# peterdavidfagan/mujoco_robot_environments

Measured on AMD Instinct MI355X. Metric: env steps/sec (whole node), RearrangementEnv batch=4096 at 1/2/4/8 MI355X, higher is better.
Workload: dtype f32

## Files before the change

mujoco_robot_environments_amd/csrc/mre_api.cpp:

```cpp
#include <hip/hip_runtime.h>
#include <chrono>

#include <cmath>
#include <cstdio>
#include <cstdlib>
#include <cstring>
#include <string>
#include <algorithm>
#include <vector>

#include "../../include/mre.h"
#include "mre_dev.h"
#include "mre_records.h"

using namespace mre;

extern "C" void mre_launch_step(const StepArgs* args, hipStream_t stream);
extern "C" void mre_launch_settle(const StepArgs* args, hipStream_t stream);
extern "C" void mre_launch_step_large(const StepArgs* args, hipStream_t stream);
extern "C" void mre_launch_step_newton(const StepArgs* args, hipStream_t stream);
extern "C" void mre_launch_settle_newton(const StepArgs* args, hipStream_t stream);
extern "C" void mre_launch_step_queue(const StepArgs* args, int nwaves, hipStream_t stream);
extern "C" void mre_launch_step_queue_newton(const StepArgs* args, int nwaves, hipStream_t stream);
extern "C" void mre_launch_step_queue_large(const StepArgs* args, int nwaves, hipStream_t stream);
// ... 87 lines not shown
  std::vector<uint8_t> h_large, h_rerun;
  int n_large = 0;
  long long* d_env_ids = nullptr;
  int *ps_attempts = nullptr, *ps_prop = nullptr, *ps_tick = nullptr, *ps_which = nullptr;
  double *ps_bounds = nullptr, *ps_pose = nullptr, *ps_zones = nullptr, *ps_pick = nullptr;
  int prop_geom0 = 12;
  int last_settle_max = 0;
  long long n_reruns = 0, n_promotions = 0, n_demotions = 0;
  struct Group {
    int lo = 0, n = 0;
    hipStream_t st = nullptr, st2 = nullptr;
    hipEvent_t ev_fork = nullptr, ev_join = nullptr;
    struct Out {
      StepArgs args;
      hipEvent_t ev_info = nullptr;
      int stage = 0;
    } out[4];
    int head = 0, nout = 0;
    int cur = 0;
    hipEvent_t p0 = nullptr, p1 = nullptr;
    int* h_order = nullptr;
    int* d_order = nullptr;
  };
  std::vector<Group> groups;
  int* h_grp_order = nullptr;
  int* d_grp_order = nullptr;
  Group qgroup;
  bool queue_ok = true;
  int queue_ticks = 200;
  int queue_waves = 0;
  int queue_shards = 16;
  int queue_lshards = 8;
  bool queue_test_serial = false;
  int queue_spare_large = 8;
  int queue_run_ticks = 100;
  int queue_min_ticks = 32;
  float tick_tail = 0.f;
  bool tick_tail_valid = false;
  float queue_tail_min = 1.45f;
  unsigned tail_samples = 0;
  std::vector<int> tail_scratch;
  int queue_large_waves_max = 0;
  int* h_qlist = nullptr;
  int* q_ws = nullptr;
  int* q_gen = nullptr;
  int* h_q_err = nullptr;
  int* h_qgrp_order = nullptr;
  long n_queue_launches = 0;
  long long n_handovers = 0;
  int queue_last_handovers = 0;
  static constexpr int RING = 4;
  int ring = 2;
  static constexpr int NSTAGE = RING + 1;
  static_assert(sizeof(Group::out) / sizeof(Group::Out) == RING, "Group::out is the ring");
  hipEvent_t ev_main = nullptr;
  float* seq_copy[RING + 1] = {nullptr, nullptr, nullptr, nullptr, nullptr};
  size_t seq_cap = 0;
  unsigned seq_calls = 0;
  double dbg_wait_s = 0, dbg_call_s = 0; long dbg_calls = 0;
  int calls_since_drain = 0, sync_streak = 0;
  bool broken = false;
};

static void launch_compact(const mre_env* e, const StepArgs& a, hipStream_t st, bool settle = false) {
  const bool newton = e->hM.solver == MRE_SOLVER_NEWTON;
  if (settle) { if (newton) mre_launch_settle_newton(&a, st); else mre_launch_settle(&a, st); }
  else { if (newton) mre_launch_step_newton(&a, st); else mre_launch_step(&a, st); }
}
static void launch_large(const mre_env* e, const StepArgs& a, hipStream_t st) {
  if (e->hM.solver == MRE_SOLVER_NEWTON) mre_launch_step_large_newton(&a, st); else mre_launch_step_large(&a, st);
}

static int profile_events(mre_env* e, hipEvent_t* e0, hipEvent_t* e1) {
  *e0 = *e1 = nullptr;
  if (!e->profiling) return MRE_OK;
  if (e->events_used == e->events.size()) {
    hipEvent_t x, y;
    HIPCHK(hipEventCreate(&x)); HIPCHK(hipEventCreate(&y));
    e->events.emplace_back(x, y);
  }
  *e0 = e->events[e->events_used].first; *e1 = e->events[e->events_used].second;
  e->events_used++;
  return MRE_OK;
}

static inline int compact_nrrow_max(const mre_env* e) {
  return e->hM.solver == MRE_SOLVER_NEWTON ? NRROW_MAX_COMPACT_NEWTON : NRROW_MAX_COMPACT_PGS;
}
static inline bool near_compact_caps(const mre_env* e, int hw_ncon, int hw_nefc, int hw_nrrow, int hw_npp) {
  return 8 * hw_ncon > 7 * NCON_MAX || 8 * hw_nefc > 7 * NEFC_MAX || 8 * hw_nrrow > 7 * compact_nrrow_max(e) || 8 * hw_npp > 7 * NPP_MAX;
}

static void sort_longest_first(const mre_env::Group& G, const int* info, int kmax, int* order_stage) {
  int count[258] = {0};
  auto bucket = [&](int i) {
    const int* li = info + 4 * (size_t)i;
    return (int)((long long)(li[0] < 0 ? 0 : (li[1] >> 16)) * 255 / kmax);
  };
  for (int i = G.lo; i < G.lo + G.n; i++) count[255 - bucket(i) + 1]++;
  for (int k = 1; k <= 256; k++) count[k] += count[k - 1];
  for (int i = G.lo; i < G.lo + G.n; i++) order_stage[G.lo + count[255 - bucket(i)]++] = i;
}
// ... 119 lines not shown
    if (rc) return rc;
  }
  return drain_group(e, e->qgroup, true);
}
#define DRAIN(e) do { int rc_ = drain(e, true); if (rc_) return rc_; } while (0)
#define DRAIN_PENDING(e) do { int rc_ = drain(e, false); if (rc_) return rc_; } while (0)

static void guard_args(mre_env* e, StepArgs& a) {
  a.large = e->d_large; a.launch_info = e->d_launch_info;
  a.sv_qpos = e->sv_qpos; a.sv_qvel = e->sv_qvel; a.sv_qacc_ws = e->sv_qacc_ws; a.sv_qfine = e->sv_qfine;
  a.sv_ctrl = e->sv_ctrl; a.sv_status = e->sv_status; a.sv_converged = e->sv_converged; a.sv_nstep = e->sv_nstep;
}

static int launch_group_enqueue(mre_env* e, mre_env::Group& G, const StepArgs& a_full, bool queue);
static int launch_group(mre_env* e, mre_env::Group& G, const StepArgs& a_full, bool queue = false) {
  const int keep = a_full.nsteps <= 50 ? e->ring - 1 : 0;
  while (G.nout > keep) {
    int rc = process_oldest(e, G);
    if (rc) return rc;
  }
  int rc = launch_group_enqueue(e, G, a_full, queue);
  if (rc) {
    (void)hipStreamSynchronize(G.st);
    (void)hipStreamSynchronize(G.st2);
    G.nout = 0; G.head = 0;
    (void)hipMemset(e->d_pending + G.lo, 0, (size_t)G.n);
    e->broken = true;
  }
  return rc;
}
static int launch_group_enqueue(mre_env* e, mre_env::Group& G, const StepArgs& a_full, bool queue) {
  int rc;
  StepArgs a = a_full;
  const size_t N = (size_t)e->N;
  if (G.nout == 0) {
    memcpy(e->h_large_stage + (size_t)G.cur * N + G.lo, e->h_large.data() + G.lo, (size_t)G.n);
    int kmax = 0;
    for (int i = G.lo; i < G.lo + G.n; i++) {
      const int* li = e->h_info_last + 4 * (size_t)i;
      if (li[0] >= 0 && (li[1] >> 16) > kmax) kmax = li[1] >> 16;
    }
    if (kmax > 0) sort_longest_first(G, e->h_info_last, kmax, G.h_order + (size_t)G.cur * N);
  }
  a.N = G.n; a.env_order = G.d_order + (size_t)G.cur * N + G.lo; a.seq_stride = e->N;
  rc = profile_events(e, &G.p0, &G.p1);
  if (rc) return rc;
  HIPCHK(hipStreamWaitEvent(G.st, e->ev_main, 0));
  if (G.p0) HIPCHK(hipEventRecord(G.p0, G.st));
  guard_args(e, a);
  a.pending = e->d_pending;
  const int slot = (G.head + G.nout) % mre_env::RING;
  a.large = e->d_large_stage + (size_t)G.cur * N;
  a.launch_info = e->d_launch_info + (size_t)slot * 4 * N;
  StepArgs ac = a;
  ac.want_large = 0;
  bool run_large = false;
  const uint8_t* const fl = e->h_large_stage + (size_t)G.cur * N;
  if (queue) {
    const int nt = a.nsteps / a.control_steps, S = e->queue_shards, cap = (G.n + S - 1) / S;
    const int SL = e->queue_lshards, capl = (G.n + SL - 1) / SL;
    constexpr int QS = QUEUE_SHARDS_MAX + QUEUE_LSHARDS_MAX;
    const size_t ctl = 2 * (size_t)QS * QUEUE_TICKS_MAX + 16;
    const size_t stride = (size_t)S * cap + (size_t)SL * capl;
    const size_t words = ctl + 4 * N + (size_t)nt * stride;
    ac.sv_qpos = nullptr;
    ac.q_head = e->q_ws; ac.q_tail = ac.q_head + QS * QUEUE_TICKS_MAX;
// ... 710 lines not shown
      e->queue_large_waves_max = 2 * prop.multiProcessorCount;
      if (const char* q = getenv("MRE_QUEUE_LSHARDS")) { const int v = atoi(q); if (v >= 1 && v <= QUEUE_LSHARDS_MAX) e->queue_lshards = v; }
      HIPCHK(hipMalloc(&e->q_ws, ((2 * (size_t)(QUEUE_SHARDS_MAX + QUEUE_LSHARDS_MAX) * QUEUE_TICKS_MAX + 16 + 4 * N +
                                   (size_t)QUEUE_TICKS_MAX * (2 * N + QUEUE_SHARDS_MAX + QUEUE_LSHARDS_MAX)) * 4 + 15) / 16 * 16));
      HIPCHK(hipMalloc(&e->q_gen, 64));
      HIPCHK(hipMemsetAsync(e->q_gen, 0, 64, e->stream));
      HIPCHK(hipHostMalloc((void**)&e->h_qlist, (size_t)(mre_env::RING + 1) * (N + 32) * 4, hipHostMallocDefault));
      HIPCHK(hipHostMalloc((void**)&e->h_q_err, 64, hipHostMallocMapped | hipHostMallocCoherent));
      *e->h_q_err = 0;
    }
    for (int g = 0; g < ng; g++) {
      auto& G = e->groups[g];
      G.h_order = e->h_grp_order; G.d_order = e->d_grp_order;
      G.lo = (int)((long long)num_envs * g / ng);
      G.n = (int)((long long)num_envs * (g + 1) / ng) - G.lo;
      int pr = 0;
      {
        int least = 0, greatest = 0;
        HIPCHK(hipDeviceGetStreamPriorityRange(&least, &greatest));
        const char* gp = getenv("MRE_GROUP_PRIORITY");
        if (!(gp && atoi(gp) == 0)) { pr = greatest + g; if (pr > least) pr = least; }
        if (const char* map = getenv("MRE_GROUP_PRIO_MAP")) {
          if ((int)strlen(map) > g && map[g] >= '0' && map[g] <= '9') { pr = greatest + (map[g] - '0'); if (pr > least) pr = least; }
        }
      }
      HIPCHK(hipStreamCreateWithPriority(&G.st, hipStreamNonBlocking, pr));
      HIPCHK(hipStreamCreateWithPriority(&G.st2, hipStreamNonBlocking, pr));
      HIPCHK(hipEventCreateWithFlags(&G.ev_fork, hipEventDisableTiming));
      HIPCHK(hipEventCreateWithFlags(&G.ev_join, hipEventDisableTiming));
      for (auto& o : G.out) HIPCHK(hipEventCreateWithFlags(&o.ev_info, hipEventDisableTiming));
    }
  }
  if (const char* fb = getenv("MRE_NO_FALLBACK")) e->fallback = atoi(fb) == 0;
  if (const char* fl = getenv("MRE_FORCE_LARGE")) {
    if (atoi(fl) != 0) {
      e->h_large.assign(N, 1); e->n_large = num_envs;
      HIPCHK(hipMemsetAsync(e->d_large, 1, N, e->stream));
    }
  }
  HIPCHK(hipMemsetAsync(e->status, 0, N * 4, e->stream)); HIPCHK(hipMemsetAsync(e->stats, 0, N * 16, e->stream));
  HIPCHK(hipMemsetAsync(e->grip_closed, 0, N, e->stream)); HIPCHK(hipMemsetAsync(e->osc_target, 0, N * 64, e->stream));
  HIPCHK(hipMemsetAsync(e->sites, 0, N * 64, e->stream));
  std::vector<int> np(N, NPROP);
  std::vector<float> ps(N * NPROP * 3, 0.0155f);
  HIPCHK(hipMemcpy(e->nprops, np.data(), N * 4, hipMemcpyHostToDevice));
  HIPCHK(hipMemcpy(e->prop_size, ps.data(), ps.size() * 4, hipMemcpyHostToDevice));
  e->osc = OscConfig{350.f, 20.f, 500.f, 100.f, 200.f, 30.f, {0.f, -0.785f, 0.f, -2.356f, 0.f, 1.571f, 0.785f},
                     5e-3f, 68e-3f, 0};
  HIPCHK(hipMalloc(&e->d_osc, sizeof(OscConfig)));
  HIPCHK(hipMemcpy(e->d_osc, &e->osc, sizeof(OscConfig), hipMemcpyHostToDevice));
  HIPCHK(hipStreamSynchronize(e->stream));
  int rc = mre_reset(e, nullptr);
  if (rc != MRE_OK) return rc;
  return mre_sync(e);
}

extern "C" int mre_create(const void* blob, size_t nbytes, int num_envs, int device_id, mre_env** out) {
  if (!blob || !out || num_envs <= 0) return fail(MRE_ERR_ARG, "mre_create: bad argument");
  *out = nullptr;
  mre_env* e = new mre_env();
  int rc = build_model(blob, nbytes, e->hM);
  if (rc != MRE_OK) { delete e; return rc; }
  if (const char* it = getenv("MRE_DEBUG_ITERS")) e->hM.iterations = atoi(it);
  e->prop_geom0 = -1;
  for (int g = 0; g < NG; g++) if (e->hM.geom_propid[g] == 0) e->prop_geom0 = g;
  if (e->prop_geom0 != PROP_GEOM0 || e->hM.geom_type[1] != 1 || e->hM.geom_body[1] != 0) {
// ... 1120 lines not shown
```

mujoco_robot_environments_amd/csrc/mre_dev.h:

```cpp
#pragma once
#include <stdint.h>

namespace mre {

constexpr int NB = 20;
constexpr int NRB = 16;
constexpr int GRIP_BODY0 = 8;
constexpr int NV = 39;
constexpr int NRV = 15;
constexpr int NQ = 43;
constexpr int NQP = 44;
constexpr int TRACE_W = 88;
constexpr int TRACE_QVEL = 48;
constexpr int NVP = 40;
constexpr int NU = 8;
constexpr int QFINE = 32;
constexpr int QFINE_ROW = 96;
constexpr int QFINE_CUBE_Q = 32;
constexpr int QFINE_CUBE_V = 60;
static_assert(QFINE_CUBE_Q + 7 * 4 == QFINE_CUBE_V && QFINE_CUBE_V + 6 * 4 <= QFINE_ROW, "qfine row layout");
constexpr int NPROP = 4;
constexpr int NG = 20;
constexpr int PROP_GEOM0 = 12;
constexpr int NPAIR = 128;
// ... 148 lines not shown
  float site_pos[NSITE][3], site_quat[NSITE][4];
  int eef_site, tcp_site;
  int eq_type[NEQ], eq_obj[NEQ][2];
  float eq_data[NEQ][8], eq_solref[NEQ][2], eq_solimp[NEQ][5];
  int ten_dof[2];
  float ten_coef[2];
  int act_dof[NU];
  float act_ctrlrange[NU][2], grip_gainprm, grip_biasprm[3], grip_forcerange[2];
  float act_gain[NU], act_bias[NU][3], act_forcerange[NU][2];
  int act_forcelimited[NU];
  float timestep, gravity[3], impratio, tolerance;
  int iterations;
  int solver;
  int cone;
  float home_qpos[7];
  float park_pos[NPROP][3];
  BodyRec body_rec[NB];
  DofRec dof_rec[NV];
  MEntryRec m_rec[NMR];
  RowRec row_rec[NROWREC];
  EqRec eq_rec[NEQ];
  SiteRec site_rec[NSITE];
  OptRec opt_rec;
};

struct OscConfig {
  float kp_pos, kd_pos, kp_ori, kd_ori, kp_null, kd_null;
  float null_q[7];
  float pos_thresh, ori_thresh;
  int pinv_always;
};

enum StepFlags : unsigned { F_NO_CONSTRAINTS = 1u, F_FREEZE_ROBOT = 2u, F_CONV_CONTINUE = 4u, F_CONV_OPEN = 8u,
                            F_OSC_EVAL = 16u, F_DETECT = 32u, F_SETTLE_EXIT = 64u };
enum CtrlMode : int { CTRL_HELD = 0, CTRL_SEQ = 1, CTRL_OSC = 2 };

struct StepArgs {
  const DevModel* M;
  int N;
  float* qpos;
  float* qvel;
  float* qacc_ws;
  float* qfine;
  float* ctrl;
  const float* ctrl_seq;
  int seq_stride;
  const int* nprops;
  const float* prop_size;
  int nsteps, control_steps, mode;
  unsigned flags;
  const OscConfig* osc;
  int osc_stride;
  const float* osc_target;
  const uint8_t* grip_closed;
  uint8_t* converged;
  float* sites;
  uint32_t* status;
  int* nstep;
  int* stats;
  float* trace;
  int trace_nenv, trace_max, trace_base;
  const uint8_t* env_mask;
  const int* env_order;
  float* geoms;
  float* contacts;
  int* settle_steps;
  int min_settle_steps;
// ... 87 lines not shown
```

mujoco_robot_environments_amd/csrc/mre_kernels.hip:

```cpp
#include <hip/hip_runtime.h>

#include "mre_dev.h"
#include "mre_math.h"
#include "mre_collide.h"

namespace mre {
using ModelP = MRE_MODEL_PTR(DevModel);
#if defined(MRE_PHASE_STAMPS) && MRE_PHASE_STAMPS >= 4
__shared__ unsigned long long dbg_acc[4];
#endif

struct OscSm {
  float J[6][7], M[7][7], MiJt[7][6], Li[6][6], Lam[6][6], V[6][6], Jbar[7][6];
  float ep[3], eo[3], F[6], LF[6], tn[7], Jbt[6], xd[6], w[6];
};

struct alignas(8) Blk {
  uint16_t row0;
  uint8_t type, nrows;
  uint8_t rslot;
  uint8_t pa, pb;
  uint8_t primary : 4;
  uint8_t bslot : 4;
};
// ... 36 lines not shown
  union { float scratch[64]; int iscr[64]; };
  float osc_tgt[16];
  int nprops;
  int ncon, nefc, nl, nrrow, npp, overflow, solver_iters;
  int finger_contact;
  uint8_t con_pair[NCON_MAX], con_rslot[NCON_MAX], con_bslot[NCON_MAX], con_b1[NCON_MAX], con_b2[NCON_MAX];
  uint16_t lim_info[NRV + 1];
  union {
    float JpA[3 * NCON_MAX][6];
    struct {
      float cinert[NB][10], crb[NRB][10], gP[NRB - GRIP_BODY0][6], gC[NRB - GRIP_BODY0][6];
      double gpose[NRB - GRIP_BODY0][7];
    };
  };
  float JpB[3 * NPP_MAX][6];
  union {
    float Jr[NRROW_MAX][NRV];
    struct {
      float cdof_dot[NV][6], cvel[NB][6], cfrc[NB][6];
      alignas(8) double gI[NRB - GRIP_BODY0][10];
      double gS[NRB - GRIP_BODY0][6];
    };
  };
#ifdef MRE_NEWTON
  float efc_R[NEFC_MAX], efc_aref[NEFC_MAX];
  float frc_r[NRROW_MAX];
  float con_fric[NCON_MAX];
  float hc[NCON_MAX][6];
  float Md[NRV][MD_LD];
  alignas(8) float W[NV * (NV + 1) / 2];
  uint8_t rstate[NEFC_MAX];
  uint8_t clist[NPROP][NCON_MAX];
  uint8_t ccount[NPROP], cpl_robot, cpl_cubes;
  alignas(8) uint16_t jdesc[NEFC_MAX][4];
  float zrow[24];
#else
  float Br[NRROW_MAX][NRV];
  alignas(16) float blkrec[MAXBLK][16];
  Blk blk[MAXBLK];
  uint8_t sched[MAXBLK][8];
#endif
  uint16_t hdr[NEFC_MAX];

  int nblk, nsched;
};

#if defined(MRE_LARGE_CAPS)
static_assert(sizeof(Sm) <= 27136, "large-capacity Sm must fit 6 workgroups per CU");
#else
static_assert(sizeof(Sm) <= 20480, "compact Sm must fit 8 workgroups per CU");
#endif

#ifdef MRE_NEWTON
MRE_DEV float* mh_store(Sm& s) { return &s.JpA[0][0]; }
static_assert(sizeof(((Sm*)0)->JpA) >= sizeof(float) * NMR, "M - h dF/dv fits the head of the constraint block");
#else
MRE_DEV float* mh_store(Sm& s) { return s.qLD; }
#endif

struct BodyRegs {
  float anchor[3], axis[3], xipos[3], ximat[9];
};

MRE_DEV double robot_q(const Sm& s, int d) { return (double)s.qpos[d] + (double)s.qlo[d]; }
MRE_DEV double robot_v(const Sm& s, int d) { return (double)s.qvel[d] + (double)s.qlo[QFINE / 2 + d]; }

// ... 1204 lines not shown
    const float v = a.qpos[(size_t)env * NQP + l];
    s.qpos[l] = v;
    if (save) a.sv_qpos[(size_t)env * NQP + l] = v;
  }
  if (l < NVP) {
    const float v = a.qvel[(size_t)env * NVP + l], w = a.qacc_ws[(size_t)env * NVP + l];
    s.qvel[l] = v;
    s.qacc[l] = w;
    s.qfrc_con[l] = 0.f;
    if (save) { a.sv_qvel[(size_t)env * NVP + l] = v; a.sv_qacc_ws[(size_t)env * NVP + l] = w; }
  }
  if (l < QFINE) {
    const float v = a.qfine != nullptr ? a.qfine[(size_t)env * QFINE_ROW + l] : 0.f;
    s.qlo[l] = v;
    if (save && a.qfine != nullptr) a.sv_qfine[(size_t)env * QFINE_ROW + l] = v;
  }
  if (save && a.qfine != nullptr && l < QFINE_ROW - QFINE)
    a.sv_qfine[(size_t)env * QFINE_ROW + QFINE + l] = a.qfine[(size_t)env * QFINE_ROW + QFINE + l];
  float cube_lo_keep = 0.f;
  if (QUEUE && !Q_LARGE && a.qfine != nullptr && l < QFINE_ROW - QFINE) cube_lo_keep = a.qfine[(size_t)env * QFINE_ROW + QFINE + l];
  if (l < NU) {
    const float v = a.ctrl[(size_t)env * NU + l];
    s.ctrl[l] = v;
    if (save) a.sv_ctrl[(size_t)env * NU + l] = v;
  }
  if (save && l == 0) {
    if (a.nstep != nullptr) a.sv_nstep[env] = a.nstep[env];
    a.sv_status[env] = a.status[env];
    a.sv_converged[env] = a.converged != nullptr ? a.converged[env] : (uint8_t)0;
  }
  if (l == 0) { s.nprops = a.nprops[env]; s.overflow = 0; s.ncon = 0; s.nefc = 0; s.solver_iters = 0; }
#ifdef MRE_NEWTON
  if (l < 24) s.zrow[l] = 0.f;
#endif
  if (l < NPROP * 3) {
    const float sz = a.prop_size[(size_t)env * NPROP * 3 + l];
    s.prop_size[l / 3][l % 3] = sz;
  }
  MRE_SYNC();
  if (l < NPROP) {
    const float m = M->body_mass[NRB + l];
    const float* z = s.prop_size[l];
    s.prop_mass[l] = m;
    s.prop_inertia[l][0] = m / 3.f * (z[1] * z[1] + z[2] * z[2]);
    s.prop_inertia[l][1] = m / 3.f * (z[0] * z[0] + z[2] * z[2]);
    s.prop_inertia[l][2] = m / 3.f * (z[0] * z[0] + z[1] * z[1]);
  }
  MRE_SYNC();

#if defined(MRE_PHASE_STAMPS) && MRE_PHASE_STAMPS >= 4
  if (l < 4) dbg_acc[l] = 0ull;
#endif
#ifdef MRE_PHASE_STAMPS
  unsigned long long stamp_acc[4] = {0, 0, 0, 0};
  unsigned long long stamp_t = __builtin_amdgcn_s_memtime();
#endif
  bool arm_converged = ((a.flags & F_CONV_CONTINUE) != 0 || (QUEUE && qtick > 0)) && a.converged != nullptr && a.converged[env] != 0;
  float grip_cmd = 0.f;
  const OscConfig* oscp = a.osc + (size_t)env * a.osc_stride;
  int hw_ncon = 0, hw_nefc = 0, hw_nrrow = 0, hw_npp = 0;
  const unsigned long long launch_t0 = __builtin_amdgcn_s_memtime();
  if (a.mode == CTRL_OSC) {
    if (l < 16) s.osc_tgt[l] = a.osc_target[(size_t)env * 16 + l];
    grip_cmd = a.grip_closed[env] ? M->act_ctrlrange[NU - 1][1] : M->act_ctrlrange[NU - 1][0];
    MRE_SYNC();
  }
// ... 566 lines not shown
```

mujoco_robot_environments_amd/csrc/mre_newton.h:

```cpp
#pragma once

namespace mre {

constexpr int NW_QUAD = 0, NW_SAT = 1, NW_CONE = 4;
constexpr int NW_LS_MAX = 20;
constexpr float NW_LS_TOL = 0.01f;
#ifndef NW_LS_REL_VALUE
#define NW_LS_REL_VALUE 1e-5f
#endif
constexpr float NW_LS_REL = NW_LS_REL_VALUE;

MRE_DEV float rdlane(float v, int lane) {
  return __builtin_bit_cast(float, __builtin_amdgcn_readlane(__builtin_bit_cast(int, v), lane));
}
MRE_DEV int uni(int v) { return __builtin_amdgcn_readfirstlane(v); }
MRE_DEV float unif(float v) {
  return __builtin_bit_cast(float, __builtin_amdgcn_readfirstlane(__builtin_bit_cast(int, v)));
}

MRE_DEV float nw_Jl(const Sm& s, int i, int h, int l, int lp, int lk) {
  const int rs = h & 0xFF, pa = (h >> 8) & 0xF, pb = (h >> 12) & 0xF;
  float j = 0.f;
  if (l < NRV) {
    if (rs != HDR_NONE) j = s.Jr[rs][l];
// ... 285 lines not shown
    const float v = s.qM[e];
    s.Md[i][j] = v; s.Md[j][i] = v;
  }
  MRE_SYNC();
  const bool on = l < NV && c.lact;
  const float fs = on ? s.qfrc_smooth[l] : 0.f, as = on ? s.qacc_smooth[l] : 0.f;
  float qa = on ? s.qacc[l] : 0.f;
  float Ma = on ? nw_mulM(s, l, c.mdiag, s.qacc) : 0.f;
  for (int i = l; i < nefc; i += 64) {
    const float aref = s.efc_aref[i];
    float d1, d2;
    row_dot2(s, i, s.qacc, s.qacc_smooth, d1, d2);
    s.jar[i] = d1 - aref;
    s.jv[i] = d2 - aref;
  }
  MRE_SYNC();
  const float gauss = wave_sum(0.5f * (Ma - fs) * (qa - as));
  const float cost_ws = gauss + nw_update<false, PYR>(s, l, nscalar, ncon, c.mu_scale, s.jar);
  const float cost_sm = nw_update<false, PYR>(s, l, nscalar, ncon, c.mu_scale, s.jv);
  if (cost_ws > cost_sm || !(cost_ws == cost_ws)) {
    qa = as; Ma = fs;
    for (int i = l; i < nefc; i += 64) s.jar[i] = s.jv[i];
  }
  if (l < NVP) { s.qacc[l] = qa; s.nw_Ma[l] = Ma; }
  MRE_SYNC();
  return nw_update_gradient<PYR>(s, l, c, nscalar, ncon);
}
MRE_PHASE_FN float nw_setup(ModelP M, Sm& s, int l) { return nw_setup_impl<false>(M, s, l); }
MRE_PHASE_FN float nw_setup_pyramidal(ModelP M, Sm& s, int l) { return nw_setup_impl<true>(M, s, l); }

MRE_PHASE_FN void nw_direction(ModelP M, Sm& s, int l) {
  MRE_DBG_T0();
  const NwLane c = nw_lane(M, s, l);
  const int nefc = s.nefc, nscalar = 7 + s.nl, nprops = s.nprops;
  const int lp = c.lp, lk = c.lk;
  float hh[NV];
#pragma unroll
  for (int k = 0; k < NV; k++) {
    float v = 0.f;
    if (k < NRV) { if (l < NRV) v = s.Md[l][k]; }
    else if (l == k) v = c.lact ? c.mdiag : 1.0f;
    hh[k] = v;
  }
  MRE_DBG_STAMP(4, 0);
#if defined(MRE_PHASE_STAMPS) && MRE_PHASE_STAMPS == 5
  {
    int nc_ = 0, nq_ = 0;
    for (int r0 = 0; r0 < nefc; r0 += 64) {
      const int st_ = r0 + l < nefc ? (int)s.rstate[r0 + l] : NW_SAT;
      nc_ += __popcll(__ballot(st_ == NW_CONE)); nq_ += __popcll(__ballot(st_ == NW_QUAD));
    }
    if (threadIdx.x == 0) { dbg_acc[2] += (unsigned long long)nc_ << 4; dbg_acc[3] += (unsigned long long)nq_ << 4; }
  }
#endif
  typedef float v4f __attribute__((ext_vector_type(4)));
  v4f c00 = {0.f, 0.f, 0.f, 0.f}, c10 = c00, c11 = c00, c20 = c00, c21 = c00, c22 = c00;
  {
    const int g = l >> 4, m16 = l & 15;
    const char* const sb = reinterpret_cast<const char*>(&s);
    const unsigned zoff = (unsigned)offsetof(Sm, zrow), jr0 = (unsigned)offsetof(Sm, Jr);
    const unsigned sh = m16 < 12 ? 16u * (unsigned)(m16 / 6) : 0u;
    const unsigned lo = 4u * (unsigned)(m16 % 6), lr = 4u * (unsigned)m16;
    auto ldw = [&](unsigned off) { return *reinterpret_cast<const float*>(sb + off); };
    auto meta = [&](int r0, int& ii, int& st, int& h, float& R, uint2& d) {
      const int i = r0 + g;
      ii = i < nefc ? i : 0;
      st = i < nefc ? (int)s.rstate[ii] : NW_SAT;
      h = s.hdr[ii];
      R = s.efc_R[ii];
      d = *reinterpret_cast<const uint2*>(&s.jdesc[ii][0]);
    };
    auto gather = [&](int h, uint2 d, float& w0, float& w1, float& w2) {
      const int rs = h & 0xFF;
      w0 = ldw((rs != HDR_NONE ? jr0 + 60u * (unsigned)rs : zoff) + lr);
      w1 = ldw(((d.x >> sh) & 0xFFFFu) + lo);
      w2 = nprops > 2 ? ldw(((d.y >> sh) & 0xFFFFu) + lo) : 0.f;
    };
    static_assert(sizeof(s.Jr[0]) == 60 && sizeof(s.JpA[0]) == 24 && sizeof(s.JpB[0]) == 24, "row strides of the gathers");
    struct Meta { int ii, st, h; float R; uint2 d; };
    auto chunk = [&](const Meta& cur, Meta& nxt, int r0) {
      const int ii = cur.ii, h = cur.h, st = cur.st;
      const uint2 d = cur.d;
      const bool quad = st == NW_QUAD, cone = st == NW_CONE;
      const float D = quad ? __builtin_amdgcn_rcpf(cur.R) : 0.f;
      if (r0 + 4 < nefc) meta(r0 + 4, nxt.ii, nxt.st, nxt.h, nxt.R, nxt.d);
      float v0, v1, v2, a0, a1, a2;
      if (__any(cone)) {
        const int cr = ii - nscalar;
        const int k = cone ? cr % 3 : 0;
        const int i0 = ii - k, i1 = cone ? i0 + 1 : ii, i2 = cone ? i0 + 2 : ii;
        float x0, x1, x2, y0, y1, y2, z0, z1, z2;
        gather(s.hdr[i0], *reinterpret_cast<const uint2*>(&s.jdesc[i0][0]), x0, x1, x2);
        gather(s.hdr[i1], *reinterpret_cast<const uint2*>(&s.jdesc[i1][0]), y0, y1, y2);
        gather(s.hdr[i2], *reinterpret_cast<const uint2*>(&s.jdesc[i2][0]), z0, z1, z2);
        const float* hcp = s.hc[cone ? cr / 3 : 0];
        const float H0 = k == 0 ? hcp[0] : (k == 1 ? hcp[1] : hcp[2]);
        const float H1 = k == 0 ? hcp[1] : (k == 1 ? hcp[3] : hcp[4]);
        const float H2 = k == 0 ? hcp[2] : (k == 1 ? hcp[4] : hcp[5]);
        v0 = k == 0 ? x0 : (k == 1 ? y0 : z0);
        v1 = k == 0 ? x1 : (k == 1 ? y1 : z1);
        v2 = k == 0 ? x2 : (k == 1 ? y2 : z2);
        a0 = cone ? H0 * x0 + H1 * y0 + H2 * z0 : v0 * D;
        a1 = cone ? H0 * x1 + H1 * y1 + H2 * z1 : v1 * D;
        a2 = cone ? H0 * x2 + H1 * y2 + H2 * z2 : v2 * D;
      } else {
        gather(h, d, v0, v1, v2);
        a0 = v0 * D; a1 = v1 * D; a2 = v2 * D;
      }
      c00 = __builtin_amdgcn_mfma_f32_16x16x4f32(a0, v0, c00, 0, 0, 0);
      c10 = __builtin_amdgcn_mfma_f32_16x16x4f32(a1, v0, c10, 0, 0, 0);
      c11 = __builtin_amdgcn_mfma_f32_16x16x4f32(a1, v1, c11, 0, 0, 0);
      if (nprops > 2) {
        c20 = __builtin_amdgcn_mfma_f32_16x16x4f32(a2, v0, c20, 0, 0, 0);
        c21 = __builtin_amdgcn_mfma_f32_16x16x4f32(a2, v1, c21, 0, 0, 0);
        c22 = __builtin_amdgcn_mfma_f32_16x16x4f32(a2, v2, c22, 0, 0, 0);
      }
    };
    Meta mA, mB;
    meta(0, mA.ii, mA.st, mA.h, mA.R, mA.d);
    mB = mA;
    for (int r0 = 0; r0 < nefc; r0 += 8) {
      chunk(mA, mB, r0);
      if (r0 + 4 < nefc) chunk(mB, mA, r0 + 4);
    }
    MRE_DBG_STAMP(4, 1);
    float* T = s.W;
    constexpr int TS = 17;
    const int mytile = l < NRV ? 0 : (l < NRV + 12 ? 1 : (l < NV ? 2 : -1));
    const int mym = l < NRV ? l : (l < NRV + 12 ? l - NRV : l - NRV - 12);
    auto spill = [&](const v4f& cv, int off) {
#pragma unroll
      for (int v = 0; v < 4; v++) T[off + (4 * g + v) * TS + m16] = cv[v];
    };
#define NW_TILE(OFF, TI, TJ, BI, NI, BJ, NJ)                                                   \
    if (mytile == TI) {                                                                        \
      _Pragma("unroll") for (int n = 0; n < NJ; n++) hh[BJ + n] += T[OFF + mym * TS + n];      \
    }                                                                                          \
    if (TI != TJ && mytile == TJ) {                                                            \
      _Pragma("unroll") for (int q = 0; q < NI; q++) hh[BI + q] += T[OFF + q * TS + mym];      \
    }
    constexpr int T2 = 16 * TS;
    static_assert(2 * T2 <= NV * (NV + 1) / 2, "two tiles fit the factor's storage");
    spill(c00, 0); spill(c10, T2);
    MRE_SYNC();
    NW_TILE(0, 0, 0, 0, NRV, 0, NRV)
    if (nprops > 0) { NW_TILE(T2, 1, 0, NRV, 12, 0, NRV) }
    MRE_SYNC();
    if (nprops > 0) {
      spill(c11, 0); spill(c20, T2);
      MRE_SYNC();
      NW_TILE(0, 1, 1, NRV, 12, NRV, 12)
      if (nprops > 2) { NW_TILE(T2, 2, 0, NRV + 12, 12, 0, NRV) }
      MRE_SYNC();
    }
    if (nprops > 2) {
      spill(c21, 0); spill(c22, T2);
      MRE_SYNC();
      NW_TILE(0, 2, 1, NRV + 12, 12, NRV, 12)
      NW_TILE(T2, 2, 2, NRV + 12, 12, NRV + 12, 12)
      MRE_SYNC();
    }
#undef NW_TILE
  }
  MRE_DBG_STAMP(4, 2);
  unsigned adj[5];
  {
    const unsigned cr = s.cpl_robot, cq = s.cpl_cubes;
    adj[0] = 0u;
#pragma unroll
    for (int p = 0; p < NPROP; p++) {
      unsigned a = (cr >> p) & 1u;
#pragma unroll
      for (int q = 0; q < NPROP; q++)
        if (q != p && ((cq >> cube_pair_bit(p, q)) & 1u)) a |= 1u << (1 + q);
      adj[1 + p] = a;
    }
#pragma unroll
    for (int a = 4; a >= 1; a--) {
      const unsigned nb = adj[a] & ((1u << a) - 1u);
#pragma unroll
      for (int b = 1; b < 4; b++)
        if (b < a && ((nb >> b) & 1u)) adj[b] |= nb & ~(1u << b);
    }
#pragma unroll
    for (int a = 1; a < 5; a++) adj[a] = (unsigned)uni((int)adj[a]);
  }
  float g = l < NVP ? s.nw_grad[l] : 0.f, y = 0.f, dinv = 1.0f;
  if (nprops > 3) nw_elim_range<NRV + 23, NRV + 18>(hh, g, y, dinv, l, adj[4] & 0xFu);
  if (nprops > 2) nw_elim_range<NRV + 17, NRV + 12>(hh, g, y, dinv, l, adj[3] & 0x7u);
  if (nprops > 1) nw_elim_range<NRV + 11, NRV + 6>(hh, g, y, dinv, l, adj[2] & 0x3u);
  if (nprops > 0) nw_elim_range<NRV + 5, NRV>(hh, g, y, dinv, l, adj[1] & 0x1u);
  nw_elim_range<NRV - 1, 0>(hh, g, y, dinv, l, 0u);
  MRE_DBG_STAMP(4, 3);
#pragma unroll
  for (int k = 0; k < NV; k++)
    if (l <= k) s.W[k * (k + 1) / 2 + l] = hh[k];
  MRE_SYNC();
  {
    const int base = l < NV ? l * (l + 1) / 2 : 0;
    const int nva = NRV + 6 * nprops;
#pragma unroll
    for (int j = 0; j < NV - 1; j++) hh[j] = (j < l && l < nva) ? s.W[base + j] : 0.f;
#pragma unroll
    for (int j = 0; j < NV - 1; j++) {
      const float xj = rdlane(y * dinv, j);
      y = fmaf(-hh[j], xj, y);
    }
  }
  const float x = (l < NV && c.lact) ? y * dinv : 0.f;
  if (l < NVP) s.nw_search[l] = -x;
  const float dec = wave_sum((l < NVP ? s.nw_grad[l] : 0.f) * x);
  if (l == 0) s.scratch[2] = dec;
  MRE_SYNC();
  MRE_DBG_STAMP(4, 3);
}

MRE_PHASE_FN void nw_direction_reuse(ModelP M, Sm& s, int l) {
  const NwLane c = nw_lane(M, s, l);
  const int nva = NRV + 6 * s.nprops;
  const bool on = l < NV && c.lact;
  const float gin = on ? s.nw_grad[l] : 0.f;
  float g = gin;
  const float dinv = on ? 1.0f / s.W[l * (l + 1) / 2 + l] : 1.0f;
  float y = 0.f;
  for (int k = nva - 1; k >= 0; k--) {
    const float yk = rdlane(g * dinv, k);
    const float w = (l < k) ? s.W[k * (k + 1) / 2 + l] : 0.f;
    g = fmaf(-w, yk, g);
    y = (l == k) ? yk : y;
  }
  const int base = l < NV ? l * (l + 1) / 2 : 0;
  for (int j = 0; j < nva; j++) {
    const float cw = (j < l && l < NV) ? s.W[base + j] : 0.f;
    const float xj = rdlane(y * dinv, j);
    y = fmaf(-cw, xj, y);
  }
  const float x = on ? y * dinv : 0.f;
  if (l < NVP) s.nw_search[l] = -x;
  const float dec = wave_sum(gin * x);
  if (l == 0) s.scratch[2] = dec;
// ... 409 lines not shown
```

Before: 23.91 million.

## Skip inactive constraint chunks and unused Hessian tiles in Newton direction

The Newton direction assembly now scans constraint rows in 64-row blocks. It builds a per-chunk mask of which Hessian block tiles each active row contributes to, and skips chunks with no quad or cone rows, so gathers and MFMAs run only for the tiles needed. Tile spills and reductions are gated on the tiles actually touched, and the factor write-back and back-substitution loops skip prop blocks beyond nprops. This adds ballot/DPP bookkeeping per block and a debug env flag to force all tiles.

```diff
diff --git a/mujoco_robot_environments_amd/csrc/mre_api.cpp b/mujoco_robot_environments_amd/csrc/mre_api.cpp
--- a/mujoco_robot_environments_amd/csrc/mre_api.cpp
+++ b/mujoco_robot_environments_amd/csrc/mre_api.cpp
@@ -143,6 +143,7 @@
   int queue_shards = 16;
   int queue_lshards = 8;
   bool queue_test_serial = false;
+  bool nw_all_tiles = false;
   int queue_spare_large = 8;
   int queue_run_ticks = 100;
   int queue_min_ticks = 32;
@@ -173,12 +174,16 @@
   bool broken = false;
 };
 
-static void launch_compact(const mre_env* e, const StepArgs& a, hipStream_t st, bool settle = false) {
+static void launch_compact(const mre_env* e, const StepArgs& a_in, hipStream_t st, bool settle = false) {
   const bool newton = e->hM.solver == MRE_SOLVER_NEWTON;
+  StepArgs a = a_in;
+  if (e->nw_all_tiles) a.flags |= F_NW_ALL_TILES;
   if (settle) { if (newton) mre_launch_settle_newton(&a, st); else mre_launch_settle(&a, st); }
   else { if (newton) mre_launch_step_newton(&a, st); else mre_launch_step(&a, st); }
 }
-static void launch_large(const mre_env* e, const StepArgs& a, hipStream_t st) {
+static void launch_large(const mre_env* e, const StepArgs& a_in, hipStream_t st) {
+  StepArgs a = a_in;
+  if (e->nw_all_tiles) a.flags |= F_NW_ALL_TILES;
   if (e->hM.solver == MRE_SOLVER_NEWTON) mre_launch_step_large_newton(&a, st); else mre_launch_step_large(&a, st);
 }
 
@@ -364,6 +369,7 @@
 static int launch_group_enqueue(mre_env* e, mre_env::Group& G, const StepArgs& a_full, bool queue) {
   int rc;
   StepArgs a = a_full;
+  if (e->nw_all_tiles) a.flags |= F_NW_ALL_TILES;
   const size_t N = (size_t)e->N;
   if (G.nout == 0) {
     memcpy(e->h_large_stage + (size_t)G.cur * N + G.lo, e->h_large.data() + G.lo, (size_t)G.n);
@@ -1140,6 +1146,7 @@
     }
   }
   if (const char* fb = getenv("MRE_NO_FALLBACK")) e->fallback = atoi(fb) == 0;
+  if (const char* q = getenv("MRE_NW_ALL_TILES")) e->nw_all_tiles = atoi(q) != 0;
   if (const char* fl = getenv("MRE_FORCE_LARGE")) {
     if (atoi(fl) != 0) {
       e->h_large.assign(N, 1); e->n_large = num_envs;
diff --git a/mujoco_robot_environments_amd/csrc/mre_dev.h b/mujoco_robot_environments_amd/csrc/mre_dev.h
--- a/mujoco_robot_environments_amd/csrc/mre_dev.h
+++ b/mujoco_robot_environments_amd/csrc/mre_dev.h
@@ -204,7 +204,7 @@
 };
 
 enum StepFlags : unsigned { F_NO_CONSTRAINTS = 1u, F_FREEZE_ROBOT = 2u, F_CONV_CONTINUE = 4u, F_CONV_OPEN = 8u,
-                            F_OSC_EVAL = 16u, F_DETECT = 32u, F_SETTLE_EXIT = 64u };
+                            F_OSC_EVAL = 16u, F_DETECT = 32u, F_SETTLE_EXIT = 64u, F_NW_ALL_TILES = 128u };
 enum CtrlMode : int { CTRL_HELD = 0, CTRL_SEQ = 1, CTRL_OSC = 2 };
 
 struct StepArgs {
diff --git a/mujoco_robot_environments_amd/csrc/mre_kernels.hip b/mujoco_robot_environments_amd/csrc/mre_kernels.hip
--- a/mujoco_robot_environments_amd/csrc/mre_kernels.hip
+++ b/mujoco_robot_environments_amd/csrc/mre_kernels.hip
@@ -92,6 +92,7 @@
   uint8_t rstate[NEFC_MAX];
   uint8_t clist[NPROP][NCON_MAX];
   uint8_t ccount[NPROP], cpl_robot, cpl_cubes;
+  uint8_t nw_all_tiles;
   alignas(8) uint16_t jdesc[NEFC_MAX][4];
   float zrow[24];
 #else
@@ -1362,6 +1363,7 @@
   if (l == 0) { s.nprops = a.nprops[env]; s.overflow = 0; s.ncon = 0; s.nefc = 0; s.solver_iters = 0; }
 #ifdef MRE_NEWTON
   if (l < 24) s.zrow[l] = 0.f;
+  if (l == 0) s.nw_all_tiles = (a.flags & F_NW_ALL_TILES) != 0 ? 1 : 0;
 #endif
   if (l < NPROP * 3) {
     const float sz = a.prop_size[(size_t)env * NPROP * 3 + l];
diff --git a/mujoco_robot_environments_amd/csrc/mre_newton.h b/mujoco_robot_environments_amd/csrc/mre_newton.h
--- a/mujoco_robot_environments_amd/csrc/mre_newton.h
+++ b/mujoco_robot_environments_amd/csrc/mre_newton.h
@@ -341,7 +341,7 @@
 MRE_PHASE_FN void nw_direction(ModelP M, Sm& s, int l) {
   MRE_DBG_T0();
   const NwLane c = nw_lane(M, s, l);
-  const int nefc = s.nefc, nscalar = 7 + s.nl, nprops = s.nprops;
+  const int nefc = uni(s.nefc), nscalar = 7 + uni(s.nl), nprops = uni(s.nprops);
   const int lp = c.lp, lk = c.lk;
   float hh[NV];
 #pragma unroll
@@ -362,8 +362,17 @@
     if (threadIdx.x == 0) { dbg_acc[2] += (unsigned long long)nc_ << 4; dbg_acc[3] += (unsigned long long)nq_ << 4; }
   }
 #endif
+#if defined(MRE_PHASE_STAMPS) && MRE_PHASE_STAMPS == 8
+  int dbg_mfma = 0, dbg_chunks = 0;
+#define NW_DBG_CHUNK(tm) do { dbg_mfma += __builtin_popcount(tm); dbg_chunks++; } while (0)
+#else
+#define NW_DBG_CHUNK(tm) do {} while (0)
+#endif
   typedef float v4f __attribute__((ext_vector_type(4)));
   v4f c00 = {0.f, 0.f, 0.f, 0.f}, c10 = c00, c11 = c00, c20 = c00, c21 = c00, c22 = c00;
+  constexpr int B00 = 1, B10 = 2, B11 = 4, B20 = 8, B21 = 16, B22 = 32;
+  constexpr int USE0 = B00 | B10 | B20, USE1 = B10 | B11 | B21, USE2 = B20 | B21 | B22;
+  int tiles = 0;
   {
     const int g = l >> 4, m16 = l & 15;
     const char* const sb = reinterpret_cast<const char*>(&s);
@@ -371,6 +380,33 @@
     const unsigned sh = m16 < 12 ? 16u * (unsigned)(m16 / 6) : 0u;
     const unsigned lo = 4u * (unsigned)(m16 % 6), lr = 4u * (unsigned)m16;
     auto ldw = [&](unsigned off) { return *reinterpret_cast<const float*>(sb + off); };
+    auto word0 = [&](int hw) { const int rs = hw & 0xFF; return ldw((rs != HDR_NONE ? jr0 + 60u * (unsigned)rs : zoff) + lr); };
+    auto word12 = [&](unsigned dw) { return ldw(((dw >> sh) & 0xFFFFu) + lo); };
+    static_assert(sizeof(s.Jr[0]) == 60 && sizeof(s.JpA[0]) == 24 && sizeof(s.JpB[0]) == 24, "row strides of the gathers");
+    const int all_tiles = uni(s.nw_all_tiles) ? (nprops > 2 ? 63 : (nprops > 0 ? B00 | B10 | B11 : B00)) : 0;
+    int tv = 0, blk = -64;
+    unsigned long long need = 0ull;
+    auto next_chunk = [&](int& r0, int& tm) {
+      while (need == 0ull) {
+        blk += 64;
+        if (blk >= nefc) { r0 = -1; tm = 0; return; }
+        const int i = blk + l, ii = i < nefc ? i : 0;
+        const int hw = s.hdr[ii], st = i < nefc ? (int)s.rstate[ii] : NW_SAT;
+        const int ra = (hw >> 8) & 0xF, rb = (hw >> 12) & 0xF;
+        const bool t0 = (hw & 0xFF) != HDR_NONE, t1 = ra < 2 || rb < 2, t2 = (ra & 0xE) == 2 || (rb & 0xE) == 2;
+        int t = (t0 ? B00 : 0) | (t1 ? B11 : 0) | (t2 ? B22 : 0) | (t0 && t1 ? B10 : 0) | (t0 && t2 ? B20 : 0) | (t1 && t2 ? B21 : 0);
+        t = (st == NW_QUAD || st == NW_CONE) ? t : 0;
+        t |= i < nefc ? all_tiles : 0;
+        t |= __builtin_amdgcn_mov_dpp(t, 0xB1, 0xF, 0xF, true);
+        t |= __builtin_amdgcn_mov_dpp(t, 0x4E, 0xF, 0xF, true);
+        tv = t;
+        need = __ballot(t != 0) & 0x1111111111111111ull;
+      }
+      const int b = __builtin_ctzll(need);
+      need &= need - 1ull;
+      r0 = blk + b;
+      tm = __builtin_amdgcn_readlane(tv, b);
+    };
     auto meta = [&](int r0, int& ii, int& st, int& h, float& R, uint2& d) {
       const int i = r0 + g;
       ii = i < nefc ? i : 0;
@@ -379,60 +415,66 @@
       R = s.efc_R[ii];
       d = *reinterpret_cast<const uint2*>(&s.jdesc[ii][0]);
     };
-    auto gather = [&](int h, uint2 d, float& w0, float& w1, float& w2) {
-      const int rs = h & 0xFF;
-      w0 = ldw((rs != HDR_NONE ? jr0 + 60u * (unsigned)rs : zoff) + lr);
-      w1 = ldw(((d.x >> sh) & 0xFFFFu) + lo);
-      w2 = nprops > 2 ? ldw(((d.y >> sh) & 0xFFFFu) + lo) : 0.f;
-    };
-    static_assert(sizeof(s.Jr[0]) == 60 && sizeof(s.JpA[0]) == 24 && sizeof(s.JpB[0]) == 24, "row strides of the gathers");
-    struct Meta { int ii, st, h; float R; uint2 d; };
-    auto chunk = [&](const Meta& cur, Meta& nxt, int r0) {
-      const int ii = cur.ii, h = cur.h, st = cur.st;
+    struct Meta { int r0, tm, ii, st, h; float R; uint2 d; };
+    auto chunk = [&](const Meta& cur, Meta& nxt) {
+      const int ii = cur.ii, h = cur.h, st = cur.st, tm = cur.tm;
       const uint2 d = cur.d;
       const bool quad = st == NW_QUAD, cone = st == NW_CONE;
       const float D = quad ? __builtin_amdgcn_rcpf(cur.R) : 0.f;
-      if (r0 + 4 < nefc) meta(r0 + 4, nxt.ii, nxt.st, nxt.h, nxt.R, nxt.d);
-      float v0, v1, v2, a0, a1, a2;
+      next_chunk(nxt.r0, nxt.tm);
+      if (nxt.r0 >= 0) meta(nxt.r0, nxt.ii, nxt.st, nxt.h, nxt.R, nxt.d);
+      tiles |= tm;
+      NW_DBG_CHUNK(tm);
+      const bool n0 = (tm & USE0) != 0, n1 = (tm & USE1) != 0, n2 = (tm & USE2) != 0;
+      float v0 = 0.f, v1 = 0.f, v2 = 0.f, a0 = 0.f, a1 = 0.f, a2 = 0.f;
       if (__any(cone)) {
         const int cr = ii - nscalar;
         const int k = cone ? cr % 3 : 0;
         const int i0 = ii - k, i1 = cone ? i0 + 1 : ii, i2 = cone ? i0 + 2 : ii;
-        float x0, x1, x2, y0, y1, y2, z0, z1, z2;
-        gather(s.hdr[i0], *reinterpret_cast<const uint2*>(&s.jdesc[i0][0]), x0, x1, x2);
-        gather(s.hdr[i1], *reinterpret_cast<const uint2*>(&s.jdesc[i1][0]), y0, y1, y2);
-        gather(s.hdr[i2], *reinterpret_cast<const uint2*>(&s.jdesc[i2][0]), z0, z1, z2);
         const float* hcp = s.hc[cone ? cr / 3 : 0];
         const float H0 = k == 0 ? hcp[0] : (k == 1 ? hcp[1] : hcp[2]);
         const float H1 = k == 0 ? hcp[1] : (k == 1 ? hcp[3] : hcp[4]);
         const float H2 = k == 0 ? hcp[2] : (k == 1 ? hcp[4] : hcp[5]);
-        v0 = k == 0 ? x0 : (k == 1 ? y0 : z0);
-        v1 = k == 0 ? x1 : (k == 1 ? y1 : z1);
-        v2 = k == 0 ? x2 : (k == 1 ? y2 : z2);
-        a0 = cone ? H0 * x0 + H1 * y0 + H2 * z0 : v0 * D;
-        a1 = cone ? H0 * x1 + H1 * y1 + H2 * z1 : v1 * D;
-        a2 = cone ? H0 * x2 + H1 * y2 + H2 * z2 : v2 * D;
+        const int h0 = s.hdr[i0], h1 = s.hdr[i1], h2 = s.hdr[i2];
+        const uint2 d0 = *reinterpret_cast<const uint2*>(&s.jdesc[i0][0]), d1 = *reinterpret_cast<const uint2*>(&s.jdesc[i1][0]),
+                    d2 = *reinterpret_cast<const uint2*>(&s.jdesc[i2][0]);
+        float x0 = 0.f, y0 = 0.f, z0 = 0.f, x1 = 0.f, y1 = 0.f, z1 = 0.f, x2 = 0.f, y2 = 0.f, z2 = 0.f;
+        if (n0) { x0 = word0(h0); y0 = word0(h1); z0 = word0(h2); }
+        if (n1) { x1 = word12(d0.x); y1 = word12(d1.x); z1 = word12(d2.x); }
+        if (n2) { x2 = word12(d0.y); y2 = word12(d1.y); z2 = word12(d2.y); }
+        if (n0) { v0 = k == 0 ? x0 : (k == 1 ? y0 : z0); a0 = cone ? H0 * x0 + H1 * y0 + H2 * z0 : v0 * D; }
+        if (n1) { v1 = k == 0 ? x1 : (k == 1 ? y1 : z1); a1 = cone ? H0 * x1 + H1 * y1 + H2 * z1 : v1 * D; }
+        if (n2) { v2 = k == 0 ? x2 : (k == 1 ? y2 : z2); a2 = cone ? H0 * x2 + H1 * y2 + H2 * z2 : v2 * D; }
       } else {
-        gather(h, d, v0, v1, v2);
+        if (n0) v0 = word0(h);
+        if (n1) v1 = word12(d.x);
+        if (n2) v2 = word12(d.y);
         a0 = v0 * D; a1 = v1 * D; a2 = v2 * D;
       }
-      c00 = __builtin_amdgcn_mfma_f32_16x16x4f32(a0, v0, c00, 0, 0, 0);
-      c10 = __builtin_amdgcn_mfma_f32_16x16x4f32(a1, v0, c10, 0, 0, 0);
-      c11 = __builtin_amdgcn_mfma_f32_16x16x4f32(a1, v1, c11, 0, 0, 0);
-      if (nprops > 2) {
-        c20 = __builtin_amdgcn_mfma_f32_16x16x4f32(a2, v0, c20, 0, 0, 0);
-        c21 = __builtin_amdgcn_mfma_f32_16x16x4f32(a2, v1, c21, 0, 0, 0);
-        c22 = __builtin_amdgcn_mfma_f32_16x16x4f32(a2, v2, c22, 0, 0, 0);
-      }
+      if (tm & B00) c00 = __builtin_amdgcn_mfma_f32_16x16x4f32(a0, v0, c00, 0, 0, 0);
+      if (tm & B10) c10 = __builtin_amdgcn_mfma_f32_16x16x4f32(a1, v0, c10, 0, 0, 0);
+      if (tm & B11) c11 = __builtin_amdgcn_mfma_f32_16x16x4f32(a1, v1, c11, 0, 0, 0);
+      if (tm & B20) c20 = __builtin_amdgcn_mfma_f32_16x16x4f32(a2, v0, c20, 0, 0, 0);
+      if (tm & B21) c21 = __builtin_amdgcn_mfma_f32_16x16x4f32(a2, v1, c21, 0, 0, 0);
+      if (tm & B22) c22 = __builtin_amdgcn_mfma_f32_16x16x4f32(a2, v2, c22, 0, 0, 0);
     };
-    Meta mA, mB;
-    meta(0, mA.ii, mA.st, mA.h, mA.R, mA.d);
-    mB = mA;
-    for (int r0 = 0; r0 < nefc; r0 += 8) {
-      chunk(mA, mB, r0);
-      if (r0 + 4 < nefc) chunk(mB, mA, r0 + 4);
+    Meta mA;
+    next_chunk(mA.r0, mA.tm);
+    meta(mA.r0 >= 0 ? mA.r0 : 0, mA.ii, mA.st, mA.h, mA.R, mA.d);
+    Meta mB = mA;
+    while (mA.r0 >= 0) {
+      chunk(mA, mB);
+      if (mB.r0 < 0) break;
+      chunk(mB, mA);
     }
     MRE_DBG_STAMP(4, 1);
+#if defined(MRE_PHASE_STAMPS) && MRE_PHASE_STAMPS == 8
+    if (threadIdx.x == 0) {
+      dbg_acc[0] += (unsigned long long)dbg_mfma << 4; dbg_acc[1] += (unsigned long long)__builtin_popcount(tiles) << 4;
+      dbg_acc[2] += (unsigned long long)dbg_chunks << 4; dbg_acc[3] += 1ull << 4;
+    }
+#endif
+#undef NW_DBG_CHUNK
     float* T = s.W;
     constexpr int TS = 17;
     const int mytile = l < NRV ? 0 : (l < NRV + 12 ? 1 : (l < NV ? 2 : -1));
@@ -450,23 +492,28 @@
     }
     constexpr int T2 = 16 * TS;
     static_assert(2 * T2 <= NV * (NV + 1) / 2, "two tiles fit the factor's storage");
-    spill(c00, 0); spill(c10, T2);
-    MRE_SYNC();
-    NW_TILE(0, 0, 0, 0, NRV, 0, NRV)
-    if (nprops > 0) { NW_TILE(T2, 1, 0, NRV, 12, 0, NRV) }
-    MRE_SYNC();
-    if (nprops > 0) {
-      spill(c11, 0); spill(c20, T2);
+    if (tiles & (B00 | B11)) {
+      if (tiles & B00) spill(c00, 0);
+      if (tiles & B11) spill(c11, T2);
       MRE_SYNC();
-      NW_TILE(0, 1, 1, NRV, 12, NRV, 12)
-      if (nprops > 2) { NW_TILE(T2, 2, 0, NRV + 12, 12, 0, NRV) }
+      if (tiles & B00) { NW_TILE(0, 0, 0, 0, NRV, 0, NRV) }
+      if (tiles & B11) { NW_TILE(T2, 1, 1, NRV, 12, NRV, 12) }
       MRE_SYNC();
     }
-    if (nprops > 2) {
-      spill(c21, 0); spill(c22, T2);
+    if (tiles & (B22 | B10)) {
+      if (tiles & B22) spill(c22, 0);
+      if (tiles & B10) spill(c10, T2);
       MRE_SYNC();
-      NW_TILE(0, 2, 1, NRV + 12, 12, NRV, 12)
-      NW_TILE(T2, 2, 2, NRV + 12, 12, NRV + 12, 12)
+      if (tiles & B22) { NW_TILE(0, 2, 2, NRV + 12, 12, NRV + 12, 12) }
+      if (tiles & B10) { NW_TILE(T2, 1, 0, NRV, 12, 0, NRV) }
+      MRE_SYNC();
+    }
+    if (tiles & (B20 | B21)) {
+      if (tiles & B20) spill(c20, 0);
+      if (tiles & B21) spill(c21, T2);
+      MRE_SYNC();
+      if (tiles & B20) { NW_TILE(0, 2, 0, NRV + 12, 12, 0, NRV) }
+      if (tiles & B21) { NW_TILE(T2, 2, 1, NRV + 12, 12, NRV, 12) }
       MRE_SYNC();
     }
 #undef NW_TILE
@@ -502,19 +549,41 @@
   nw_elim_range<NRV - 1, 0>(hh, g, y, dinv, l, 0u);
   MRE_DBG_STAMP(4, 3);
 #pragma unroll
-  for (int k = 0; k < NV; k++)
+  for (int k = 0; k < NRV; k++)
     if (l <= k) s.W[k * (k + 1) / 2 + l] = hh[k];
+#pragma unroll
+  for (int p = 0; p < NPROP; p++)
+    if (nprops > p) {
+#pragma unroll
+      for (int k = NRV + 6 * p; k < NRV + 6 * p + 6; k++)
+        if (l <= k) s.W[k * (k + 1) / 2 + l] = hh[k];
+    }
   MRE_SYNC();
   {
     const int base = l < NV ? l * (l + 1) / 2 : 0;
     const int nva = NRV + 6 * nprops;
 #pragma unroll
-    for (int j = 0; j < NV - 1; j++) hh[j] = (j < l && l < nva) ? s.W[base + j] : 0.f;
-#pragma unroll
-    for (int j = 0; j < NV - 1; j++) {
+    for (int j = 0; j < NRV; j++) hh[j] = (j < l && l < nva) ? s.W[base + j] : 0.f;
+#pragma unroll
+    for (int p = 0; p < NPROP; p++)
+      if (nprops > p) {
+#pragma unroll
+        for (int j = NRV + 6 * p; j < NRV + 6 * p + 6 && j < NV - 1; j++) hh[j] = (j < l && l < nva) ? s.W[base + j] : 0.f;
+      }
+#pragma unroll
+    for (int j = 0; j < NRV; j++) {
       const float xj = rdlane(y * dinv, j);
       y = fmaf(-hh[j], xj, y);
     }
+#pragma unroll
+    for (int p = 0; p < NPROP; p++)
+      if (nprops > p) {
+#pragma unroll
+        for (int j = NRV + 6 * p; j < NRV + 6 * p + 6 && j < NV - 1; j++) {
+          const float xj = rdlane(y * dinv, j);
+          y = fmaf(-hh[j], xj, y);
+        }
+      }
   }
   const float x = (l < NV && c.lact) ? y * dinv : 0.f;
   if (l < NVP) s.nw_search[l] = -x;
```

After: 24.28 million, median of 6. 1.02x the previous value.
